# esologic/GANce

Measured on AMD Instinct MI355X. Metric: synthesized frames/sec at 1024x1024 config-f, higher is better.
Workload: dtype f32 (bf16x3 split operands, 6 terms, fp32 accumulate)

## Files before the change

gance_amd/csrc/winograd43_conv.hip:

```cpp

#include <hip/hip_runtime.h>

#include <algorithm>
#include <cstdint>
#include <cstdio>
#include <cstdlib>

#include "kernels.h"

#ifndef GANCE_W43_WINDOW
#define GANCE_W43_WINDOW 0
#endif
#ifndef GANCE_W43_ABLATE
#define GANCE_W43_ABLATE 0
#endif

namespace gance {

namespace {

typedef float f32x4 __attribute__((ext_vector_type(4)));
typedef float f32x2 __attribute__((ext_vector_type(2)));
typedef __attribute__((address_space(3))) void* lds_ptr_t;

constexpr int kKC = 4;
#ifndef GANCE_W43_ODD_SHIFT
#define GANCE_W43_ODD_SHIFT 0
#endif
constexpr int kOddShift = GANCE_W43_ODD_SHIFT;
constexpr int kBM = 32;
constexpr int kUnit = 16 * 36;
constexpr int kWPieces = 18;
constexpr int kWFloats = kWPieces * 256;
constexpr int kPiecesPerWave = 5;
template <int TW>
struct Geo43 {
    static constexpr int kTW = TW, kTH = 1024 / TW;
    static constexpr int kTC = TW / 4, kTR = 16 / kTC;
    static constexpr int kPW = kTW + 8, kPH = kTH + 2;
    static constexpr int kPlane = kPH * kPW;
    static constexpr int kPatchF4 = kKC * kPlane / 4;
    static constexpr int kPPieces = (kPatchF4 + 63) / 64;
    static constexpr int kPieces = kWPieces + kPPieces;
    static_assert(kPieces <= 8 * kPiecesPerWave && kPieces > 7 * kPiecesPerWave, "five LDS-DMA pieces per wave and chunk");
    static constexpr int kSlot = kPieces * 256;
    static constexpr int kNoiseRowsPerPiece = 256 / kTW;
};
#ifndef GANCE_W43_NBUF
#define GANCE_W43_NBUF 3
#endif
constexpr int kNBUF = GANCE_W43_NBUF;
constexpr int kConstD = 0, kConstB = 64, kConstS = 128, kConstNoise = 192, kConstRgb = kConstNoise + 1024, kConstFloats = kConstRgb + 512;
constexpr int kStoresPerEpilogue = 16, kRgbStores = 12;
constexpr int kRgbXchgFloats = 4 * 12 * 16 * 4;

template <typename T>
__device__ __forceinline__ void input_transform6(T d0, T d1, T d2, T d3, T d4, T d5, T (&t)[6]) {
    const T a = d4 - 4.f * d2;
    const T b = d3 - 4.f * d1;
    const T c = d4 - d2;
    const T e = d3 - d1;
    t[0] = 4.f * d0 + (d4 - 5.f * d2);
    t[1] = a + b;
    t[2] = a - b;
    t[3] = c + 2.f * e;
    t[4] = c - 2.f * e;
    t[5] = 4.f * d1 + (d5 - 5.f * d3);
}

__device__ __forceinline__ void input_transform6_row(f32x2 r05, f32x2 r12, f32x2 r34, float (&t)[6]) {
    const f32x2 ba = r34 - 4.f * r12;
    const f32x2 ec = r34 - r12;
    f32x2 t12, t34;
    asm("v_pk_add_f32 %0, %1, %1 op_sel:[1,0] op_sel_hi:[1,0] neg_hi:[0,1]" : "=v"(t12) : "v"(ba));
    asm("v_pk_fma_f32 %0, %1, 2.0, %1 op_sel:[0,0,1] op_sel_hi:[0,0,1] neg_hi:[1,0,0]" : "=v"(t34) : "v"(ec));
    t[0] = 4.f * r05[0] + (r34[1] - 5.f * r12[1]);
    t[1] = t12[0];
    t[2] = t12[1];
    t[3] = t34[0];
    t[4] = t34[1];
    t[5] = 4.f * r12[0] + (r05[1] - 5.f * r34[0]);
}

__device__ __forceinline__ void output_transform6(float m0, float m1, float m2, float m3, float m4, float m5, float (&y)[4]) {
    const float s1 = m1 + m2, d1 = m1 - m2, s2 = m3 + m4, d2 = m3 - m4;
    y[0] = m0 + s1 + s2;
    y[1] = fmaf(2.f, d2, d1);
    y[2] = fmaf(4.f, s2, s1);
    y[3] = fmaf(8.f, d2, d1) + m5;
}

struct Tile43 {
    int m_tile, y0, x0, b0;
};

__device__ __forceinline__ int fresh_lane() {
    int l;
    asm volatile("v_mbcnt_lo_u32_b32 %0, -1, 0\n\tv_mbcnt_hi_u32_b32 %0, -1, %0" : "=v"(l));
    return l;
}

}

template <bool RGB, int TW>
__device__ __forceinline__ void winograd43_body(const ConvArgs& p) {
    using Geo = Geo43<TW>;
    constexpr int kTW = Geo::kTW, kTH = Geo::kTH, kPW = Geo::kPW, kPH = Geo::kPH, kPlane = Geo::kPlane, kPatchF4 = Geo::kPatchF4;
    constexpr int kPieces = Geo::kPieces, kSlot = Geo::kSlot, kTC = Geo::kTC, kTR = Geo::kTR;
    extern __shared__ __attribute__((aligned(16))) float smem[];
    float* const const0 = smem + kNBUF * kSlot;
    const int tid = threadIdx.x;
    const int wave = __builtin_amdgcn_readfirstlane(tid >> 6);
    __shared__ int simd_tickets[4];
    if (tid < 4) simd_tickets[tid] = 0;
    __syncthreads();
    const int pg = __builtin_amdgcn_s_getreg((1 << 11) | (4 << 6) | 4) & 3;
    int ticket = 0;
    if ((tid & 63) == 0) ticket = atomicAdd(&simd_tickets[pg], 1) & 1;
    const int cot = __builtin_amdgcn_readfirstlane(ticket);
    const int role = cot;
    __syncthreads();
    if (simd_tickets[0] != 2 || simd_tickets[1] != 2 || simd_tickets[2] != 2 || simd_tickets[3] != 2) {
        if (wave == 0 && fresh_lane() == 0 && p.fault_flag != nullptr) __hip_atomic_store(p.fault_flag, 43, __ATOMIC_RELAXED, __HIP_MEMORY_SCOPE_SYSTEM);
        return;
    }
    const int Hp = p.H + 2, Wp = p.W + 8;
    const int n = p.total_chunks;
    const int my_tiles = (p.total_tiles - (int)blockIdx.x + (int)gridDim.x - 1) / (int)gridDim.x;
    const int total = my_tiles * n;

    auto decode = [&](int i) {
        const int v = (int)blockIdx.x + i * (int)gridDim.x;
        const int nwg = p.total_tiles;
        const int q = nwg >> 3, r = nwg & 7, xcd = v & 7;
        int id = (xcd < r ? xcd * (q + 1) : r * (q + 1) + (xcd - r) * q) + (v >> 3);
        Tile43 t;
        if (p.m_tiles == 16 && p.xcd_blocking) {
            const int j = id & 63, sg = id >> 6;
            t.m_tile = 8 * (j >> 5) + (j & 7);
            id = 4 * sg + ((j & 31) >> 3);
        } else {
            t.m_tile = id % p.m_tiles;
            id /= p.m_tiles;
        }
        t.x0 = (id % p.tiles_x) * kTW;
        id /= p.tiles_x;
        t.y0 = (id % p.tiles_y) * kTH;
        t.b0 = id / p.tiles_y;
        return t;
    };

    const __amdgpu_buffer_rsrc_t w_rsrc = __builtin_amdgcn_make_buffer_rsrc((void*)p.w, 0, 0x7fffffff, 0x00020000);
    int piece_voff[kPiecesPerWave];
    int win_off, a_off;
    auto lane_setup = [&]() {
        const int lane = fresh_lane();
        const int n16 = lane & 15, g = lane >> 4;
#pragma unroll
        for (int r = 0; r < kPiecesPerWave; ++r) {
            int piece = wave * kPiecesPerWave + r;
            if (piece >= kPieces) piece = kWPieces;
            if (piece < kWPieces) {
                piece_voff[r] = piece * 1024 + lane * 16;
            } else {
                int f = (piece - kWPieces) * 64 + lane;
                if (f >= kPatchF4) f = (piece - kWPieces) * 64;
                const int q4 = f % (kPW / 4);
                const int row = (f / (kPW / 4)) % kPH;
                const int c = f / (kPW / 4 * kPH);
                piece_voff[r] = ((c * Hp + row) * Wp + 4 * q4 - kOddShift * (c & 1)) * 4;
            }
        }
        win_off = kWFloats + g * kPlane + 4 * (pg * kTR + n16 / kTC) * kPW + 4 * (n16 % kTC) + kOddShift * (g & 1);
        a_off = (cot * 4 + g) * kUnit + n16 * 36;
    };
    lane_setup();
    int st_tile = 0, st_q = 0, st_slot = 0, st_w = 0, st_x = 0, st_count = 0;
    __amdgpu_buffer_rsrc_t st_x_rsrc = w_rsrc;
    const int x_chunk_step = kKC * Hp * Wp * 4;
    int cur_slot = 0, cur_w = 0, cur_x = 0;
    bool cur_valid = false;
    auto stage_begin = [&]() {
        cur_valid = st_count < total;
        if (!cur_valid) return;
        if (st_q == 0) {
            const Tile43 t = decode(st_tile);
            const int lane = fresh_lane();
            st_x_rsrc = __builtin_amdgcn_make_buffer_rsrc((void*)(p.x + (size_t)t.b0 * p.x_b_stride), 0, 0x7fffffff, 0x00020000);
            st_w = t.m_tile * n * (kWFloats * 4);
            st_x = (t.y0 * Wp + t.x0) * 4;
            float* const set = const0 + (st_tile & 1) * kConstFloats;
            const int co = t.m_tile * kBM;
            if (wave < 3) {
                const float* src = wave == 0 ? p.d + (size_t)t.b0 * p.d_stride + co
                                             : (wave == 1 ? p.bias + co : (p.s_next != nullptr ? p.s_next + (size_t)t.b0 * p.s_stride + co : nullptr));
                if (src != nullptr) {
                    const __amdgpu_buffer_rsrc_t c_rsrc = __builtin_amdgcn_make_buffer_rsrc((void*)src, 0, kBM * 4, 0x00020000);
                    __builtin_amdgcn_raw_ptr_buffer_load_lds(c_rsrc, (lds_ptr_t)(set + wave * 64), 4, lane * 4, 0, 0, 0);
                }
            } else if (wave < 7) {
                if (p.noise != nullptr) {
                    const __amdgpu_buffer_rsrc_t nz_rsrc = __builtin_amdgcn_make_buffer_rsrc((void*)p.noise, 0, 0x7fffffff, 0x00020000);
                    const int row = Geo::kNoiseRowsPerPiece * (wave - 3) + lane / kTC;
                    __builtin_amdgcn_raw_ptr_buffer_load_lds(nz_rsrc, (lds_ptr_t)(set + kConstNoise + (wave - 3) * 256), 16,
                                                             ((t.y0 + row) * p.OW + t.x0 + 4 * (lane % kTC)) * 4, t.b0 * p.noise_b_stride * 4, 0, 0);
                }
            } else if (RGB) {
                const __amdgpu_buffer_rsrc_t a_rsrc = __builtin_amdgcn_make_buffer_rsrc(
                    (void*)(p.rgb_coef + ((size_t)t.b0 * (p.Cout / 4) + 8 * t.m_tile) * 64), 0, 512 * 4, 0x00020000);
                __builtin_amdgcn_raw_ptr_buffer_load_lds(a_rsrc, (lds_ptr_t)(set + kConstRgb), 16, lane * 16, 0, 0, 0);
                __builtin_amdgcn_raw_ptr_buffer_load_lds(a_rsrc, (lds_ptr_t)(set + kConstRgb + 256), 16, lane * 16, 1024, 0, 0);
            }
        }
        cur_slot = st_slot;
        cur_w = st_w;
        cur_x = st_x;
        st_w += kWFloats * 4;
        st_x += x_chunk_step;
        st_slot = st_slot == kNBUF - 1 ? 0 : st_slot + 1;
        ++st_count;
        if (++st_q == n) {
            st_q = 0;
            ++st_tile;
        }
    };
    auto stage_piece = [&](int r) {
        float* const base = smem + cur_slot * kSlot;
        int piece = wave * kPiecesPerWave + r;
        if (piece >= kPieces) piece = kWPieces;
        if (piece < kWPieces)
            __builtin_amdgcn_raw_ptr_buffer_load_lds(w_rsrc, (lds_ptr_t)(base + piece * 256), 16, piece_voff[r], cur_w, 0, 0);
        else
            __builtin_amdgcn_raw_ptr_buffer_load_lds(st_x_rsrc, (lds_ptr_t)(base + kWFloats + (piece - kWPieces) * 256), 16, piece_voff[r], cur_x, 0, 0);
    };

    float* const rgb_xchg = const0 + 2 * kConstFloats;

    f32x4 acc[36];

    float V[36], A[36];
#if GANCE_W43_ABLATE & 12
    for (int k = 0; k < 36; ++k) V[k] = A[k] = 0.f;
#endif
    auto load_transform = [&](int slot) {
        const float* const P = smem + slot * kSlot + win_off;
        const float* const U = smem + slot * kSlot + a_off;
#if GANCE_W43_ABLATE & 8
#pragma unroll
        for (int k = 0; k < 36; ++k) asm volatile("" : "+v"(V[k]));
#if GANCE_W43_ABLATE & 4
#pragma unroll
        for (int k = 0; k < 36; ++k) asm volatile("" : "+v"(A[k]));
#else
#pragma unroll
        for (int k = 0; k < 9; ++k) {
            const f32x4 t = *reinterpret_cast<const f32x4*>(U + 4 * k);
            A[4 * k + 0] = t[0], A[4 * k + 1] = t[1], A[4 * k + 2] = t[2], A[4 * k + 3] = t[3];
        }
#endif
        return;
#endif
        f32x2 c45[6], c67[6], c38[6];
#pragma unroll
        for (int y = 0; y < 6; ++y) {
#if GANCE_W43_WINDOW == 1
            const f32x4 q0 = *reinterpret_cast<const f32x4*>(P + y * kPW);
            const f32x4 q1 = *reinterpret_cast<const f32x4*>(P + y * kPW + 4);
            const f32x4 q2 = *reinterpret_cast<const f32x4*>(P + y * kPW + 8);
            c45[y] = f32x2{q1[0], q1[1]};
            c67[y] = f32x2{q1[2], q1[3]};
            c38[y] = f32x2{q0[3], q2[0]};
#else
            c45[y] = *reinterpret_cast<const f32x2*>(P + y * kPW + 4);
            c67[y] = *reinterpret_cast<const f32x2*>(P + y * kPW + 6);
#if GANCE_W43_WINDOW == 3
            c38[y][0] = (*reinterpret_cast<const f32x2*>(P + y * kPW + 2))[1];
            c38[y][1] = (*reinterpret_cast<const f32x2*>(P + y * kPW + 8))[0];
#else
            c38[y][0] = P[y * kPW + 3];
            c38[y][1] = P[y * kPW + 8];
#endif
#endif
        }
#if GANCE_W43_ABLATE & 4
#pragma unroll
        for (int k = 0; k < 36; ++k) asm volatile("" : "+v"(A[k]));
#else
#pragma unroll
        for (int k = 0; k < 9; ++k) {
            const f32x4 t = *reinterpret_cast<const f32x4*>(U + 4 * k);
            A[4 * k + 0] = t[0];
            A[4 * k + 1] = t[1];
            A[4 * k + 2] = t[2];
            A[4 * k + 3] = t[3];
        }
#endif
#if GANCE_W43_ABLATE & 2
#pragma unroll
        for (int y = 0; y < 6; ++y) {
            V[y * 6 + 0] = c38[y][0], V[y * 6 + 1] = c45[y][0], V[y * 6 + 2] = c45[y][1];
            V[y * 6 + 3] = c67[y][0], V[y * 6 + 4] = c67[y][1], V[y * 6 + 5] = c38[y][1];
        }
        return;
#endif
        f32x2 t45[6], t67[6], t38[6];
        input_transform6<f32x2>(c45[0], c45[1], c45[2], c45[3], c45[4], c45[5], t45);
        input_transform6<f32x2>(c67[0], c67[1], c67[2], c67[3], c67[4], c67[5], t67);
        input_transform6<f32x2>(c38[0], c38[1], c38[2], c38[3], c38[4], c38[5], t38);
#pragma unroll
        for (int i = 0; i < 6; ++i) {
            asm("" : "+v"(t45[i]), "+v"(t67[i]), "+v"(t38[i]));
            float v[6];
            input_transform6_row(t38[i], t45[i], t67[i], v);
#pragma unroll
            for (int j = 0; j < 6; ++j) V[j * 6 + i] = v[j];
        }
    };
    auto multiply = [&](auto first_tag) {
        constexpr bool kFirst = decltype(first_tag)::value;
#pragma unroll
        for (int pos = 0; pos < 36; ++pos) {
            acc[pos] = __builtin_amdgcn_mfma_f32_16x16x4f32(A[pos], V[pos], kFirst ? f32x4{0.f, 0.f, 0.f, 0.f} : acc[pos], 0, 0, 0);
            if (pos % 7 == 3 && cur_valid && !(GANCE_W43_ABLATE & 1)) stage_piece(pos / 7);
        }
        __builtin_amdgcn_sched_group_barrier(0x008, 4, 0);
        __builtin_amdgcn_sched_group_barrier(0x020, 1, 0);
#pragma unroll
        for (int i = 0; i < 4; ++i) {
            __builtin_amdgcn_sched_group_barrier(0x008, 7, 0);
            __builtin_amdgcn_sched_group_barrier(0x020, 1, 0);
        }
        __builtin_amdgcn_sched_group_barrier(0x008, 4, 0);
    };

    auto epilogue = [&](int i) {
        const Tile43 t = decode(i);
        const float* const set = const0 + (i & 1) * kConstFloats;
        const int lane = fresh_lane();
        const int n16 = lane & 15, g = lane >> 4;
        const int ty4 = 4 * (pg * kTR + n16 / kTC), tx4 = 4 * (n16 % kTC);
        const int oy0 = t.y0 + ty4, ox0 = t.x0 + tx4;
        const int ct = t.m_tile * 2 + cot;
        const int co0 = ct * 16 + 4 * g;
        const f32x4 dm = *reinterpret_cast<const f32x4*>(set + kConstD + cot * 16 + 4 * g);
        const f32x4 bm = *reinterpret_cast<const f32x4*>(set + kConstB + cot * 16 + 4 * g);
        f32x4 sn = f32x4{1.f, 1.f, 1.f, 1.f};
        if (p.s_next != nullptr) sn = *reinterpret_cast<const f32x4*>(set + kConstS + cot * 16 + 4 * g);
        f32x4 rgbacc[4][4];
        if constexpr (RGB) {
#pragma unroll
            for (int oy = 0; oy < 4; ++oy)
#pragma unroll
                for (int ox = 0; ox < 4; ++ox) rgbacc[oy][ox] = f32x4{0.f, 0.f, 0.f, 0.f};
        }
        float* const out_base = p.out == nullptr ? nullptr
                                                 : p.out + (size_t)t.b0 * p.out_b_stride + (size_t)co0 * p.out_c_stride +
                                                       (size_t)(oy0 + p.out_y_off) * p.out_row_stride + ox0 + p.out_x_off;
#pragma unroll
        for (int r = 0; r < 4; ++r) {
            __builtin_amdgcn_sched_barrier(0);
            float a_rgb = 0.f;
            if constexpr (RGB) a_rgb = set[kConstRgb + (cot * 4 + r) * 64 + lane] * 1.4142135623730951f;
            const float s2 = sn[r] * 1.4142135623730951f;
            float tr[4][6];
#pragma unroll
            for (int j = 0; j < 6; ++j) {
                float col[4];
                output_transform6(acc[j * 6 + 0][r], acc[j * 6 + 1][r], acc[j * 6 + 2][r], acc[j * 6 + 3][r], acc[j * 6 + 4][r], acc[j * 6 + 5][r], col);
#pragma unroll
                for (int oy = 0; oy < 4; ++oy) tr[oy][j] = col[oy];
            }
#pragma unroll
            for (int oy = 0; oy < 4; ++oy) {
                float yrow[4];
                output_transform6(tr[oy][0], tr[oy][1], tr[oy][2], tr[oy][3], tr[oy][4], tr[oy][5], yrow);
                f32x4 nz = f32x4{0.f, 0.f, 0.f, 0.f};
                if (p.noise != nullptr) nz = *reinterpret_cast<const f32x4*>(set + kConstNoise + (ty4 + oy) * kTW + tx4) * p.noise_strength;
                f32x4 v = f32x4{yrow[0], yrow[1], yrow[2], yrow[3]} * dm[r] + nz + bm[r];
#pragma unroll
                for (int k = 0; k < 4; ++k) v[k] = fmaxf(v[k], 0.2f * v[k]);
                if constexpr (RGB) {
#pragma unroll
                    for (int ox = 0; ox < 4; ++ox) rgbacc[oy][ox] = __builtin_amdgcn_mfma_f32_16x16x4f32(a_rgb, v[ox], rgbacc[oy][ox], 0, 0, 0);
                }
                if (out_base != nullptr) *reinterpret_cast<f32x4*>(out_base + (size_t)r * p.out_c_stride + (size_t)oy * p.out_row_stride) = v * s2;
            }
        }
        __builtin_amdgcn_sched_barrier(0);
        if constexpr (RGB) {
            f32x4* const xchg = reinterpret_cast<f32x4*>(rgb_xchg) + (pg * 12) * 16 + n16;
            if (cot == 0) {
                if (g == 0) {
#pragma unroll
                    for (int c = 0; c < 3; ++c)
#pragma unroll
                        for (int oy = 0; oy < 4; ++oy) xchg[(c * 4 + oy) * 16] = f32x4{rgbacc[oy][0][c], rgbacc[oy][1][c], rgbacc[oy][2][c], rgbacc[oy][3][c]};
                }
                asm volatile("s_waitcnt lgkmcnt(0)" ::: "memory");
            } else if (g == 0) {
                float* const y_base = p.rgb_y + (((size_t)t.m_tile * p.B + t.b0) * 3) * p.OH * p.OW + (size_t)oy0 * p.OW + ox0;
#pragma unroll
                for (int c = 0; c < 3; ++c)
#pragma unroll
                    for (int oy = 0; oy < 4; ++oy)
                        *reinterpret_cast<f32x4*>(y_base + ((size_t)c * p.OH + oy) * p.OW) =
                            f32x4{rgbacc[oy][0][c], rgbacc[oy][1][c], rgbacc[oy][2][c], rgbacc[oy][3][c]} + xchg[(c * 4 + oy) * 16];
            }
        }
        lane_setup();
    };

    for (int c = 0; c < kNBUF - 1; ++c) {
        stage_begin();
        if (cur_valid) {
#pragma unroll
            for (int r = 0; r < kPiecesPerWave; ++r) stage_piece(r);
        }
    }

    int slot = 0, G = 0;
    auto open_interval = [&](bool stores_behind, bool rgb_stores = false) {
        if (G + 1 >= total)
            asm volatile("s_waitcnt vmcnt(0)" ::: "memory");
        else if (stores_behind && rgb_stores)
            asm volatile("s_waitcnt vmcnt(%0)" ::"n"(kPiecesPerWave + kStoresPerEpilogue + kRgbStores) : "memory");
        else if (stores_behind)
            asm volatile("s_waitcnt vmcnt(%0)" ::"n"(kPiecesPerWave + kStoresPerEpilogue) : "memory");
        else
            asm volatile("s_waitcnt vmcnt(%0)" ::"n"(kPiecesPerWave) : "memory");
        if (!(GANCE_W43_ABLATE & 16)) __builtin_amdgcn_s_barrier();
        asm volatile("" ::: "memory");
        stage_begin();
        __builtin_amdgcn_sched_barrier(0);
    };
    auto close_interval = [&]() {
        __builtin_amdgcn_sched_barrier(0);
        slot = slot == kNBUF - 1 ? 0 : slot + 1;
        ++G;
    };
    if (role == 0) {
        int tile = 0;
        do {
            open_interval(tile > 0);
            load_transform(slot);
            __builtin_amdgcn_sched_barrier(0);
            multiply(std::true_type{});
            close_interval();
            int q = 1;
            do {
                open_interval(false);
                load_transform(slot);
                __builtin_amdgcn_sched_barrier(0);
                multiply(std::false_type{});
                close_interval();
            } while (++q < n);
            epilogue(tile);
        } while (++tile < my_tiles);
        if constexpr (RGB) __builtin_amdgcn_s_barrier();
    } else {
        open_interval(false);
        if (cur_valid) {
#pragma unroll
            for (int r = 0; r < kPiecesPerWave; ++r) stage_piece(r);
        }
        load_transform(slot);
        close_interval();
        int tile = 0;
        do {
            open_interval(tile > 0, RGB);
            multiply(std::true_type{});
            __builtin_amdgcn_sched_barrier(0);
            load_transform(slot);
            close_interval();
            int q = 2;
            do {
                open_interval(false);
                multiply(std::false_type{});
                __builtin_amdgcn_sched_barrier(0);
                load_transform(slot);
                close_interval();
            } while (++q < n);
            const bool more = tile + 1 < my_tiles;
            if (more) {
                open_interval(false);
            } else {
                cur_valid = false;
                if constexpr (RGB) __builtin_amdgcn_s_barrier();
            }
            multiply(std::false_type{});
            __builtin_amdgcn_sched_barrier(0);
            epilogue(tile);
            if (more) {
                load_transform(slot);
                close_interval();
            }
        } while (++tile < my_tiles);
    }
    asm volatile("s_waitcnt vmcnt(0)" ::: "memory");
}

__global__ __launch_bounds__(512, 1) void winograd43_kernel(const ConvArgs p) { winograd43_body<false, 64>(p); }
__global__ __launch_bounds__(512, 1) void winograd43_rgb_kernel(const ConvArgs p) { winograd43_body<true, 64>(p); }
__global__ __launch_bounds__(512, 1) void winograd43_w32_kernel(const ConvArgs p) { winograd43_body<false, 32>(p); }
__global__ __launch_bounds__(512, 1) void winograd43_w32_rgb_kernel(const ConvArgs p) { winograd43_body<true, 32>(p); }

bool winograd43_supported(int cin, int cout, int H, int W) {
    return cin % kKC == 0 && cin / kKC >= 4 && cout % kBM == 0 && ((W % 64 == 0 && H % 16 == 0) || (W == 32 && H % 32 == 0));
}

size_t winograd43_weight_floats(int cin, int cout) { return (size_t)(cout / kBM) * (cin / kKC) * kWFloats; }

bool winograd43_rgb_supported(int cout) { return winograd64_rgb_supported(cout); }
int winograd43_rgb_partials(int cout) { return cout / kBM; }

void winograd43_transform_weights(const float* w_in, int cin, int cout, float* w_out) {
    const double G[6][3] = {{1. / 4, 0., 0.},          {-1. / 6, -1. / 6, -1. / 6}, {-1. / 6, 1. / 6, -1. / 6},
                            {1. / 24, 1. / 12, 1. / 6}, {1. / 24, -1. / 12, 1. / 6}, {0., 0., 1.}};
    const int chunks = cin / kKC;
    std::fill(w_out, w_out + winograd43_weight_floats(cin, cout), 0.f);
    for (int co = 0; co < cout; ++co)
        for (int ci = 0; ci < cin; ++ci) {
            double gk[3][3], tmp[6][3], u[6][6];
            for (int ky = 0; ky < 3; ++ky)
                for (int kx = 0; kx < 3; ++kx) gk[ky][kx] = w_in[((size_t)(ky * 3 + kx) * cin + ci) * cout + co];
            for (int i = 0; i < 6; ++i)
                for (int kx = 0; kx < 3; ++kx) tmp[i][kx] = G[i][0] * gk[0][kx] + G[i][1] * gk[1][kx] + G[i][2] * gk[2][kx];
            for (int i = 0; i < 6; ++i)
                for (int j = 0; j < 6; ++j) u[i][j] = tmp[i][0] * G[j][0] + tmp[i][1] * G[j][1] + tmp[i][2] * G[j][2];
            const int mtile = co / kBM, m = co % kBM, ch = ci / kKC, kc = ci % kKC;
            float* dst = w_out + ((size_t)mtile * chunks + ch) * kWFloats + ((m / 16) * 4 + kc) * kUnit + (m % 16) * 36;
            for (int i = 0; i < 6; ++i)
                for (int j = 0; j < 6; ++j) dst[j * 6 + i] = (float)u[i][j];
        }
}

hipError_t launch_winograd43_conv(const ConvArgs& args, hipStream_t stream) {
    const bool rgb = args.epilogue == kEpilogueFullRgbPart;
    if (!winograd43_supported(args.Cin, args.Cout, args.H, args.W)) return hipErrorInvalidValue;
    if (rgb ? (!winograd43_rgb_supported(args.Cout) || args.rgb_coef == nullptr || args.rgb_y == nullptr) : (args.epilogue != kEpilogueFull || args.out == nullptr))
        return hipErrorInvalidValue;
    const bool narrow = args.W % 64 != 0;
    void (*const kernel)(const ConvArgs) = narrow ? (rgb ? winograd43_w32_rgb_kernel : winograd43_w32_kernel) : (rgb ? winograd43_rgb_kernel : winograd43_kernel);
    const int tw = narrow ? 32 : 64, th = 1024 / tw;
    const size_t lds_bytes = sizeof(float) * ((size_t)kNBUF * (narrow ? Geo43<32>::kSlot : Geo43<64>::kSlot) + 2 * kConstFloats + (rgb ? kRgbXchgFloats : 0));
    static PerDeviceInt resident[4];
    int resident_blocks = 0;
    hipError_t e = resident[(narrow ? 2 : 0) + (rgb ? 1 : 0)].get(
        [&](int device, int* value) {
            hipError_t err = hipFuncSetAttribute(reinterpret_cast<const void*>(kernel), hipFuncAttributeMaxDynamicSharedMemorySize, (int)lds_bytes);
            if (err != hipSuccess) return err;
            int cus = 0;
            if ((err = hipDeviceGetAttribute(&cus, hipDeviceAttributeMultiprocessorCount, device)) != hipSuccess) return err;
            *value = std::max(8, cus / 8 * 8);
            return hipSuccess;
        },
        &resident_blocks);
    if (e != hipSuccess) return e;
    ConvArgs a = args;
    a.tiles_x = a.W / tw;
    a.tiles_y = a.H / th;
    a.m_tiles = a.Cout / kBM;
    a.total_chunks = a.Cin / kKC;
    a.total_tiles = a.m_tiles * a.tiles_x * a.tiles_y * a.B;
    if ((a.tiles_x * a.tiles_y * a.B) % 4 != 0) a.xcd_blocking = 0;
    int rounds = std::max(1, a.grid_rounds);
    const int min_tiles = std::max(1, 64 / a.total_chunks);
    while (rounds > 1 && a.total_tiles < resident_blocks * rounds * min_tiles) --rounds;
    hipLaunchKernelGGL(kernel, dim3(std::min(a.total_tiles, resident_blocks * rounds)), dim3(512), lds_bytes, stream, a);
    return hipGetLastError();
}

}
```

Before: 1463.

## Defer ToRGB partial reduction and overlap role-0 epilogue with next tile's multiply

Measured after the change: 1483, median of 6. 1.01x the previous value.

```diff
diff --git a/gance_amd/csrc/winograd43_conv.hip b/gance_amd/csrc/winograd43_conv.hip
--- a/gance_amd/csrc/winograd43_conv.hip
+++ b/gance_amd/csrc/winograd43_conv.hip
@@ -235,6 +235,7 @@
     };
 
     float* const rgb_xchg = const0 + 2 * kConstFloats;
+    size_t rgb_off = 0;
 
     f32x4 acc[36];
 
@@ -388,26 +389,33 @@
         }
         __builtin_amdgcn_sched_barrier(0);
         if constexpr (RGB) {
-            f32x4* const xchg = reinterpret_cast<f32x4*>(rgb_xchg) + (pg * 12) * 16 + n16;
-            if (cot == 0) {
-                if (g == 0) {
-#pragma unroll
-                    for (int c = 0; c < 3; ++c)
-#pragma unroll
-                        for (int oy = 0; oy < 4; ++oy) xchg[(c * 4 + oy) * 16] = f32x4{rgbacc[oy][0][c], rgbacc[oy][1][c], rgbacc[oy][2][c], rgbacc[oy][3][c]};
-                }
-                asm volatile("s_waitcnt lgkmcnt(0)" ::: "memory");
-            } else if (g == 0) {
-                float* const y_base = p.rgb_y + (((size_t)t.m_tile * p.B + t.b0) * 3) * p.OH * p.OW + (size_t)oy0 * p.OW + ox0;
+            f32x4* const xchg = reinterpret_cast<f32x4*>(rgb_xchg + cot * kRgbXchgFloats) + (pg * 12) * 16 + n16;
+            if (g == 0) {
 #pragma unroll
                 for (int c = 0; c < 3; ++c)
 #pragma unroll
-                    for (int oy = 0; oy < 4; ++oy)
-                        *reinterpret_cast<f32x4*>(y_base + ((size_t)c * p.OH + oy) * p.OW) =
-                            f32x4{rgbacc[oy][0][c], rgbacc[oy][1][c], rgbacc[oy][2][c], rgbacc[oy][3][c]} + xchg[(c * 4 + oy) * 16];
-            }
+                    for (int oy = 0; oy < 4; ++oy) xchg[(c * 4 + oy) * 16] = f32x4{rgbacc[oy][0][c], rgbacc[oy][1][c], rgbacc[oy][2][c], rgbacc[oy][3][c]};
+            }
+            asm volatile("s_waitcnt lgkmcnt(0)" ::: "memory");
+            rgb_off = (((size_t)t.m_tile * p.B + t.b0) * 3) * p.OH * p.OW + (size_t)t.y0 * p.OW + t.x0;
         }
         lane_setup();
+    };
+    auto finish_rgb = [&]() {
+        const int lane = fresh_lane();
+        const int n16 = lane & 15;
+        if (lane < 16) {
+            const f32x4* const x0 = reinterpret_cast<const f32x4*>(rgb_xchg) + (pg * 12) * 16 + n16;
+            const f32x4* const x1 = x0 + kRgbXchgFloats / 4;
+            float* const y_base = p.rgb_y + rgb_off + (size_t)(4 * (pg * kTR + n16 / kTC)) * p.OW + 4 * (n16 % kTC);
+#pragma unroll
+            for (int c = 0; c < 3; ++c) {
+#pragma unroll
+                for (int oy = 0; oy < 4; ++oy)
+                    *reinterpret_cast<f32x4*>(y_base + ((size_t)c * p.OH + oy) * p.OW) = x1[(c * 4 + oy) * 16] + x0[(c * 4 + oy) * 16];
+                __builtin_amdgcn_sched_barrier(0);
+            }
+        }
     };
 
     for (int c = 0; c < kNBUF - 1; ++c) {
@@ -419,13 +427,13 @@
     }
 
     int slot = 0, G = 0;
-    auto open_interval = [&](bool stores_behind, bool rgb_stores = false) {
+    auto open_interval = [&](int stores) {
         if (G + 1 >= total)
             asm volatile("s_waitcnt vmcnt(0)" ::: "memory");
-        else if (stores_behind && rgb_stores)
-            asm volatile("s_waitcnt vmcnt(%0)" ::"n"(kPiecesPerWave + kStoresPerEpilogue + kRgbStores) : "memory");
-        else if (stores_behind)
+        else if (stores == kStoresPerEpilogue)
             asm volatile("s_waitcnt vmcnt(%0)" ::"n"(kPiecesPerWave + kStoresPerEpilogue) : "memory");
+        else if (stores == kRgbStores)
+            asm volatile("s_waitcnt vmcnt(%0)" ::"n"(kPiecesPerWave + kRgbStores) : "memory");
         else
             asm volatile("s_waitcnt vmcnt(%0)" ::"n"(kPiecesPerWave) : "memory");
         if (!(GANCE_W43_ABLATE & 16)) __builtin_amdgcn_s_barrier();
@@ -438,27 +446,52 @@
         slot = slot == kNBUF - 1 ? 0 : slot + 1;
         ++G;
     };
+    const int act_stores = p.out != nullptr ? kStoresPerEpilogue : 0;
     if (role == 0) {
+        lane_setup();
+        open_interval(0);
+        load_transform(slot);
+        __builtin_amdgcn_sched_barrier(0);
+        multiply(std::true_type{});
+        close_interval();
         int tile = 0;
+        int stores = 0, stores_next = 0;
         do {
-            open_interval(tile > 0);
-            load_transform(slot);
-            __builtin_amdgcn_sched_barrier(0);
-            multiply(std::true_type{});
-            close_interval();
             int q = 1;
             do {
-                open_interval(false);
+                open_interval(stores);
+                if constexpr (RGB) {
+                    if (stores_next != 0) finish_rgb();
+                }
+                stores = stores_next;
+                stores_next = 0;
+                asm volatile("" : "+s"(stores), "+s"(stores_next));
                 load_transform(slot);
                 __builtin_amdgcn_sched_barrier(0);
                 multiply(std::false_type{});
                 close_interval();
             } while (++q < n);
+            const bool more = tile + 1 < my_tiles;
+            if (more)
+                open_interval(0);
+            else
+                cur_valid = false;
             epilogue(tile);
+            stores = act_stores;
+            stores_next = RGB ? kRgbStores : 0;
+            if (more) {
+                load_transform(slot);
+            } else {
+#pragma unroll
+                for (int k = 0; k < 36; ++k) asm volatile("" : "=v"(V[k]), "=v"(A[k]));
+            }
+            __builtin_amdgcn_sched_barrier(0);
+            multiply(std::true_type{});
+            if (more) close_interval();
         } while (++tile < my_tiles);
-        if constexpr (RGB) __builtin_amdgcn_s_barrier();
     } else {
-        open_interval(false);
+        lane_setup();
+        open_interval(0);
         if (cur_valid) {
 #pragma unroll
             for (int r = 0; r < kPiecesPerWave; ++r) stage_piece(r);
@@ -467,26 +500,24 @@
         close_interval();
         int tile = 0;
         do {
-            open_interval(tile > 0, RGB);
+            open_interval(tile > 0 ? act_stores : 0);
             multiply(std::true_type{});
             __builtin_amdgcn_sched_barrier(0);
             load_transform(slot);
             close_interval();
             int q = 2;
             do {
-                open_interval(false);
+                open_interval(0);
                 multiply(std::false_type{});
                 __builtin_amdgcn_sched_barrier(0);
                 load_transform(slot);
                 close_interval();
             } while (++q < n);
             const bool more = tile + 1 < my_tiles;
-            if (more) {
-                open_interval(false);
-            } else {
+            if (more)
+                open_interval(0);
+            else
                 cur_valid = false;
-                if constexpr (RGB) __builtin_amdgcn_s_barrier();
-            }
             multiply(std::false_type{});
             __builtin_amdgcn_sched_barrier(0);
             epilogue(tile);
@@ -495,6 +526,11 @@
                 close_interval();
             }
         } while (++tile < my_tiles);
+    }
+    if constexpr (RGB) {
+        __builtin_amdgcn_s_barrier();
+        asm volatile("" ::: "memory");
+        if (role == 0) finish_rgb();
     }
     asm volatile("s_waitcnt vmcnt(0)" ::: "memory");
 }
@@ -542,7 +578,9 @@
     const bool narrow = args.W % 64 != 0;
     void (*const kernel)(const ConvArgs) = narrow ? (rgb ? winograd43_w32_rgb_kernel : winograd43_w32_kernel) : (rgb ? winograd43_rgb_kernel : winograd43_kernel);
     const int tw = narrow ? 32 : 64, th = 1024 / tw;
-    const size_t lds_bytes = sizeof(float) * ((size_t)kNBUF * (narrow ? Geo43<32>::kSlot : Geo43<64>::kSlot) + 2 * kConstFloats + (rgb ? kRgbXchgFloats : 0));
+    const size_t lds_bytes = sizeof(float) * ((size_t)kNBUF * (narrow ? Geo43<32>::kSlot : Geo43<64>::kSlot) + 2 * kConstFloats + (rgb ? 2 * kRgbXchgFloats : 0));
+    static_assert(sizeof(float) * (kNBUF * std::max(Geo43<32>::kSlot, Geo43<64>::kSlot) + 2 * kConstFloats + 2 * kRgbXchgFloats) + 64 <= 160 * 1024 || kNBUF != 3,
+                  "ring + tile constants + ToRGB buffers must fit the LDS of a CU");
     static PerDeviceInt resident[4];
     int resident_blocks = 0;
     hipError_t e = resident[(narrow ? 2 : 0) + (rgb ? 1 : 0)].get(
```
